# tuna2134/sbv2-api

Hardware: NVIDIA B200
Metric: audio-sec/sec (higher is better)
Workload: dtype f16 operands / f32 accumulate on tcgen05 (decoder, flow; text encoder with two-term fp16 splits); f32 elsewhere

## Files before the change

### sbv2-api_b200/csrc/umma_conv.h

```cpp
#pragma once
#include <cuda_fp16.h>

#include <map>
#include <vector>

#include "common.h"
#include "kernels.h"

struct sbv2_model;

namespace sbv2 {

constexpr int UMMA_GAP = 32;
constexpr int UMMA_TAIL_ROWS = 2304;
constexpr int UMMA_MAX_TAPS = 16;
constexpr int UMMA_MAX_GROUPS = 8;

struct HostConv {
  std::vector<float> w, b;
  int d0 = 0, d1 = 0, k = 1;
};

struct DecoderHostWeights {
  HostConv pre, cond, post;
  std::vector<HostConv> ups;
  std::vector<int> up_u;
  std::vector<std::vector<HostConv>> res_c1, res_c2;
  std::vector<std::vector<int>> res_dil;
  int per = 3;
  int gin = 512;
};

struct ConvLayer {
  __half* w = nullptr;
  float* bias = nullptr;
  int cin = 0, cout = 0, nb = 0, n_nblk = 1, taps = 1, kc = 64, nkc = 1, mt = 1, sps = 1, nstages = 2, nloads = 1, total_steps = 1;
  int a_slots = 1;
  int b_resident = 0;
  int n_groups = 1;
  int tap_shift[UMMA_MAX_GROUPS][UMMA_MAX_TAPS] = {{0}};
  int group_out_off[UMMA_MAX_GROUPS] = {0};
  int halo_lo = 0, halo_hi = 0;
  size_t smem = 0;
  int tmem_cols = 32;
  unsigned idesc = 0;
  float in_scale = 1.f, out_scale = 1.f;
};

ConvLayer make_conv1d_layer(sbv2_model* owner, const HostConv& c, int dil, int mt_pref, int nb_max = 256);
ConvLayer make_gated_conv1d_layer(sbv2_model* owner, const HostConv& c, int dil, int mt_pref, int* gate_half, std::vector<int>* perm);
ConvLayer make_upsample_layer(sbv2_model* owner, const HostConv& c, int u, int mt_pref);

struct Geom {
  int mul = 1;
  long long rows_tot = 0;
  std::vector<int> pstart, len;
  const int* d_pstart = nullptr;
  const int* d_len = nullptr;
  const int* d_prefix[5] = {nullptr, nullptr, nullptr, nullptr, nullptr};
  int n_tiles[5] = {0, 0, 0, 0, 0};
  std::map<int, std::pair<const int*, int>> extra;
  int max_len = 0;
};
struct BatchGeom {
  std::vector<Geom> g;
  const int* d_ystart = nullptr;
  const int* d_wstart = nullptr;
  const int* d_order = nullptr;
};
struct DBuf;
struct PinnedBuf;
BatchGeom build_geoms(sbv2_model* owner, DBuf& dev, PinnedBuf& pin, const std::vector<int>& ystart, const std::vector<int>& ylen,
                      const std::vector<int>& muls, const std::vector<std::vector<int>>* extra_heights = nullptr, bool pin_idle = false,
                      const std::vector<long long>* wstart = nullptr );

ConvLayer make_split_conv1d_layer(sbv2_model* owner, const HostConv& c, int dil, int mt_pref, int terms, int nb_max = 256);
void launch_split_planar(const LaunchCtx& ctx, __half* out, const float* in, int in_ld, int C, const int* d_start, const Geom& g,
                         int n_utt, int terms, float in_scale);
enum UAccum { UACC_NONE = 0, UACC_SET = 1, UACC_ADD = 2, UACC_FINAL = 3 };
struct ConvCall {
  const __half* in = nullptr;
  __half* out = nullptr;
  const __half* residual = nullptr;
  const __half* residual2 = nullptr;
  const __half* residual3 = nullptr;
  float out_div = 1.f;
  float* accum = nullptr;
  int accum_mode = UACC_NONE;
  float accum_div = 1.f;
  int act_out = ACT_NONE;
  bool act_on_accum = false;
  const float* bias_utt = nullptr;
  int bias_utt_ld = 0;
  int gate_half = 0;
  int out_mul = 1, out_off = 0;
  float* rm_out = nullptr;
  int rm_ld = 0;
  const int* rm_start = nullptr;
  __half* split_out = nullptr;
  float split_scale = 16.f;
  bool tmap = false;
  int cluster = 0;
  bool pair = false;
  bool splitk = false;
};
void launch_umma(const LaunchCtx& ctx, const ConvLayer& L, const Geom& gi, const Geom& go, const ConvCall& c, int n_utt);
void launch_zero_gaps(const LaunchCtx& ctx, __half* buf, int C, const Geom& g, int n_utt);
void launch_planar_cast(const LaunchCtx& ctx, __half* out, const float* in, int C, const Geom& g, int n_utt);
void launch_to_planar(const LaunchCtx& ctx, __half* out, const float* in, int in_ld, int C, const int* d_start, const Geom& g,
                      int n_utt, int act);
void launch_from_planar(const LaunchCtx& ctx, float* out, const __half* in, int C, const int* d_start, const Geom& g, int n_utt);

struct PairLayer {
  __half* w1 = nullptr;
  __half* w2 = nullptr;
  float* bias1 = nullptr;
  float* bias2 = nullptr;
  int c = 0, taps = 1, kc = 16, nkc = 1, mt = 1, t1rows = 128, t1pitch = 144, out_rows = 128, h1 = 0, h2 = 0;
  int shift1[UMMA_MAX_TAPS] = {0};
  int sps = 1, nstages = 1, nloads = 1, total_steps = 1, a_slots = 2, b_resident = 0;
  size_t smem = 0;
  int tmem_cols = 512;
  unsigned idesc = 0;
};
struct PairCall {
  const __half* in = nullptr;
  __half* out = nullptr;
  const __half* residual2 = nullptr;
  const __half* residual3 = nullptr;
  float out_div = 1.f;
  int act_out = ACT_LRELU;
};
bool make_pair_layer(sbv2_model* owner, const HostConv& c1, int dil, const HostConv& c2, PairLayer* out);
void launch_umma_pair(const LaunchCtx& ctx, const PairLayer& L, const Geom& g, const PairCall& c, int n_utt);

struct UmmaDecoder;
UmmaDecoder* umma_decoder_create(const DecoderHostWeights& w, sbv2_model* owner);
void umma_decoder_free(UmmaDecoder* d);
void umma_decoder_run(UmmaDecoder* d, sbv2_model* owner, const float* z, const float* g, int B,
                      const std::vector<int>& ystart, const std::vector<int>& ylen, float* wave,
                      const std::vector<long long>* wstart = nullptr);

}
```

### sbv2-api_b200/csrc/umma_pair.cu

```cuda
#include <cuda_fp16.h>

#include <algorithm>
#include <cstdlib>

#include "kernels.h"
#include "model.h"
#include "umma_conv.h"
#include "umma_device.cuh"

namespace sbv2 {
namespace {

constexpr int P_MAX_ASLOTS = 8, P_MAX_STAGES = 4, P_EPI_WARPS = 16, P_THREADS = 64 + 32 * P_EPI_WARPS + 32;
constexpr int P_B_PRODUCER_WARP = 2 + P_EPI_WARPS;
constexpr int P_SMEM_LIMIT = 227 * 1024;

struct PairArgs {
  __half* out;
  long long out_plane_stride;
  const __half* residual;
  const __half* residual2;
  const __half* residual3;
  float out_div;
  float* accum;
  int accum_mode, act_on_accum;
  float accum_div;
  int act_out;
  float act_slope;
  const __half* in;
  const __half* w1;
  const __half* w2;
  const float* bias1;
  const float* bias2;
  const int* tile_prefix;
  const int* pstart;
  const int* len;
  int n_utt, n_items;
  int c, taps, kc, nkc, mt, t1rows, t1pitch, out_rows, h1, h2;
  int shift1[UMMA_MAX_TAPS];
  int sps, nstages, nloads, total_steps, a_slots, b_resident;
  int has_res;
  int tmem_cols;
  unsigned idesc;
  long long* trace;
};

#define PTRACE(ev, itv)                                                                          \
  do {                                                                                            \
    if (p.trace != nullptr && blockIdx.x == 0 && (itv) < 64) p.trace[(itv) * 16 + (ev)] = clock64(); \
  } while (0)

struct PTile {
  int b, t0, len, pstart;
};
constexpr int P_TABLE_UTTS = 128;
struct PTables {
  const int* prefix;
  const int* len;
  const int* pstart;
};
__device__ __forceinline__ PTile locate_pair_item(const PairArgs& p, const PTables& tb, int item) {
  PTile ti;
  int lo = 0, hi = p.n_utt;
  while (hi - lo > 1) {
    const int mid = (lo + hi) >> 1;
    if (tb.prefix[mid] <= item) lo = mid;
    else hi = mid;
  }
  ti.b = lo;
  ti.t0 = (item - tb.prefix[lo]) * p.out_rows;
  ti.len = tb.len[lo];
  ti.pstart = tb.pstart[lo];
  return ti;
}

template <int C>
struct PairShape {
  static constexpr int c = C, mt = 128 / C, kc = C < 64 ? C : 64, nkc = C / kc, t1rows = 128 * mt, t1pitch = t1rows + 16;
};

template <int C>
__global__ void __launch_bounds__(P_THREADS, 1) umma_pair_kernel(const __grid_constant__ PairArgs p) {
  using K = PairShape<C>;
  extern __shared__ __align__(128) uint8_t smem[];
  const int warp = __shfl_sync(0xffffffffu, (int)(threadIdx.x >> 5), 0), lane = threadIdx.x & 31;
  const int RA = K::t1rows + 2 * p.h1;
  const int ppc = K::kc / 8;
  const uint32_t slot_bytes = (uint32_t)ppc * RA * 16;
  const uint32_t step_bytes = (uint32_t)K::c * K::kc * 2;
  const uint32_t stage_bytes = step_bytes * p.sps;
  const uint32_t t1_bytes = (uint32_t)(K::c / 8) * K::t1pitch * 16;
  const uint32_t sA = smem_u32(smem);
  const uint32_t sT1 = sA + ((slot_bytes * p.a_slots + 127u) & ~127u);
  const uint32_t sB = sT1 + 2 * t1_bytes;
  const uint32_t sBar = sB + (p.b_resident ? 2 * step_bytes * p.total_steps : stage_bytes * p.nstages);
  const uint32_t bar_af = sBar, bar_ae = bar_af + 8 * P_MAX_ASLOTS, bar_bf = bar_ae + 8 * P_MAX_ASLOTS, bar_be = bar_bf + 8 * P_MAX_STAGES,
                 bar_a1f = bar_be + 8 * P_MAX_STAGES, bar_a1e = bar_a1f + 16, bar_a2f = bar_a1e + 16, bar_a2e = bar_a2f + 16,
                 bar_t1r = bar_a2e + 16, bar_t1f = bar_t1r + 16;
  const uint32_t tmem_slot = bar_t1f + 16;
  volatile uint32_t* tmem_slot_ptr = reinterpret_cast<volatile uint32_t*>(smem + (tmem_slot - sA));
  float* bias_s = reinterpret_cast<float*>(smem + (sBar - sA) + 384);
  const int acc_cols = K::mt * K::c;

  if (threadIdx.x == 0) {
    for (int i = 0; i < p.a_slots; ++i) {
      mbar_init(bar_af + 8 * i, 1);
      mbar_init(bar_ae + 8 * i, 1);
    }
    for (int i = 0; i < P_MAX_STAGES; ++i) {
      mbar_init(bar_bf + 8 * i, 1);
      mbar_init(bar_be + 8 * i, 1);
    }
    for (int i = 0; i < 2; ++i) {
      mbar_init(bar_a1f + 8 * i, 1);
      mbar_init(bar_a1e + 8 * i, P_EPI_WARPS);
      mbar_init(bar_a2f + 8 * i, 1);
      mbar_init(bar_a2e + 8 * i, P_EPI_WARPS);
      mbar_init(bar_t1r + 8 * i, P_EPI_WARPS);
      mbar_init(bar_t1f + 8 * i, 1);
    }
    asm volatile("fence.mbarrier_init.release.cluster;" ::: "memory");
  }
  for (int i = threadIdx.x; i < 2 * K::c; i += P_THREADS) bias_s[i] = i < K::c ? p.bias1[i] : p.bias2[i - K::c];
  PTables tb{p.tile_prefix, p.len, p.pstart};
  if (p.n_utt <= P_TABLE_UTTS) {
    int* tab = reinterpret_cast<int*>(bias_s + 2 * K::c);
    for (int i = threadIdx.x; i <= p.n_utt; i += P_THREADS) tab[i] = p.tile_prefix[i];
    for (int i = threadIdx.x; i < p.n_utt; i += P_THREADS) {
      tab[p.n_utt + 1 + i] = p.len[i];
      tab[2 * p.n_utt + 1 + i] = p.pstart[i];
    }
    tb.prefix = tab;
    tb.len = tab + p.n_utt + 1;
    tb.pstart = tab + 2 * p.n_utt + 1;
  }
  if (warp == 1) {
    asm volatile("tcgen05.alloc.cta_group::1.sync.aligned.shared::cta.b32 [%0], %1;" ::"r"(tmem_slot), "r"((uint32_t)p.tmem_cols) : "memory");
    asm volatile("tcgen05.relinquish_alloc_permit.cta_group::1.sync.aligned;" ::: "memory");
  }
  tc_fence_before();
  __syncthreads();
  tc_fence_after();
  const uint32_t tmem_base = *tmem_slot_ptr;
  pdl_launch_dependents();
  pdl_wait();
  const int n_my = p.n_items > (int)blockIdx.x ? (p.n_items - 1 - (int)blockIdx.x) / (int)gridDim.x + 1 : 0;

  if (warp == 0) {
    if (lane == 0) {
      uint32_t a_it = 0;
      auto load_a_item = [&](int it) {
        const PTile ti = locate_pair_item(p, tb, (int)blockIdx.x + it * (int)gridDim.x);
        const long long in_row0 = (long long)ti.pstart + ti.t0 - p.h2 - p.h1;
        for (int kc = 0; kc < K::nkc; ++kc, ++a_it) {
          const uint32_t slot = a_it % p.a_slots;
          mbar_wait(bar_ae + 8 * slot, ((a_it / p.a_slots) & 1) ^ 1);
          mbar_expect_tx(bar_af + 8 * slot, slot_bytes);
          for (int q = 0; q < ppc; ++q) {
            const int plane = kc * ppc + q;
            bulk_g2s(sA + slot_bytes * slot + (uint32_t)q * RA * 16, p.in + (size_t)plane * p.out_plane_stride + in_row0 * 8, (uint32_t)RA * 16,
                     bar_af + 8 * slot);
          }
        }
      };
      for (int it = 0; it < n_my; ++it) load_a_item(it);
    }
  } else if (warp == P_B_PRODUCER_WARP) {
    if (lane == 0) {
      uint32_t b_it = 0;
      auto load_b_all = [&](const __half* w) {
        for (int i = 0; i < p.nloads; ++i, ++b_it) {
          const uint32_t st = b_it % p.nstages;
          mbar_wait(bar_be + 8 * st, ((b_it / p.nstages) & 1) ^ 1);
          const int first_step = i * p.sps;
          const int nsteps = min(p.sps, p.total_steps - first_step);
          const uint32_t bytes = step_bytes * nsteps;
          mbar_expect_tx(bar_bf + 8 * st, bytes);
          bulk_g2s(sB + stage_bytes * st, w + (size_t)first_step * (step_bytes / 2), bytes, bar_bf + 8 * st);
        }
      };
      if (p.b_resident && n_my > 0) {
        const uint32_t wb = step_bytes * p.total_steps;
        mbar_expect_tx(bar_bf, 2 * wb);
        bulk_g2s(sB, p.w1, wb, bar_bf);
        bulk_g2s(sB + wb, p.w2, wb, bar_bf);
      }
      if (!p.b_resident) {
        if (n_my > 0) load_b_all(p.w1);
        for (int it = 0; it < n_my; ++it) {
          if (it + 1 < n_my) load_b_all(p.w1);
          load_b_all(p.w2);
        }
      }
    }
  } else if (warp == 1) {
    const int k16 = K::kc / 16, mt = K::mt;
    const uint32_t c_u = (uint32_t)K::c, idesc = p.idesc;
    const uint64_t desc_hi = (uint64_t)(0x4000u | (128u >> 4)) << 32;
    const uint64_t a_desc0 = desc_hi | ((uint64_t)((uint32_t)RA & 0x3FFF) << 16);
    const uint64_t t_desc0 = desc_hi | ((uint64_t)((uint32_t)K::t1pitch & 0x3FFF) << 16);
    const uint64_t b_desc0 = desc_hi | ((uint64_t)((uint32_t)K::c & 0x3FFF) << 16);
    const uint32_t a_kstep = 2u * (uint32_t)RA, t_kstep = 2u * (uint32_t)K::t1pitch, b_kstep = 2u * (uint32_t)K::c;
    uint32_t a_slot_i = 0, a_par = 0, b_st = 0, b_par = 0;
    int b_si = 0;
    bool resident_ready = false;
    auto b_step_addr = [&](int conv, int step) -> uint32_t {
      if (p.b_resident) {
        if (!resident_ready) {
          mbar_wait(bar_bf, 0);
          resident_ready = true;
        }
        return sB + (uint32_t)conv * step_bytes * p.total_steps + step_bytes * step;
      }
      if (b_si == 0) mbar_wait(bar_bf + 8 * b_st, b_par);
      return sB + stage_bytes * b_st + step_bytes * b_si;
    };
    const bool leader = elect_one_sync() != 0;
    auto b_step_done = [&](int step) {
      if (p.b_resident) return;
      ++b_si;
      if (b_si == p.sps || step == p.total_steps - 1) {
        if (leader) tc_commit(bar_be + 8 * b_st);
        b_si = 0;
        if (++b_st == (uint32_t)p.nstages) {
          b_st = 0;
          b_par ^= 1;
        }
      }
    };
    auto issue_p1 = [&](int it, auto mtk) {
      constexpr int MT = decltype(mtk)::mt, K16 = decltype(mtk)::k16;
      const uint32_t buf = it & 1;
      mbar_wait(bar_a1e + 8 * buf, ((it >> 1) & 1) ^ 1);
      tc_fence_after();
      if (lane == 0) PTRACE(0, it);
      const uint32_t tacc0 = tmem_base + buf * acc_cols;
      int step = 0;
      for (int kc = 0; kc < K::nkc; ++kc) {
        mbar_wait(bar_af + 8 * a_slot_i, a_par);
        const uint64_t a_chunk = a_desc0 + ((sA + slot_bytes * a_slot_i) >> 4) + (uint32_t)p.h1;
        for (int tap = 0; tap < p.taps; ++tap, ++step) {
          const uint32_t b_addr = b_step_addr(0, step);
          const uint64_t a_tap = a_chunk + (int64_t)p.shift1[tap];
          const uint64_t b_d = b_desc0 + (b_addr >> 4);
          const uint32_t accf = step > 0 ? 1u : 0u;
          if (leader) issue_mmas<MT, K16>(tacc0, a_tap, b_d, a_kstep, b_kstep, c_u, idesc, accf);
          b_step_done(step);
        }
        if (leader) tc_commit(bar_ae + 8 * a_slot_i);
        if (++a_slot_i == (uint32_t)p.a_slots) {
          a_slot_i = 0;
          a_par ^= 1;
        }
      }
      if (leader) tc_commit(bar_a1f + 8 * buf);
      __syncwarp();
      if (lane == 0) PTRACE(1, it);
    };
    auto issue_p2 = [&](int it, auto mtk) {
      constexpr int MT = decltype(mtk)::mt, K16 = decltype(mtk)::k16;
      const uint32_t buf = it & 1;
      if (lane == 0) PTRACE(8, it);
      mbar_wait(bar_a2e + 8 * buf, ((it >> 1) & 1) ^ 1);
      if (lane == 0) PTRACE(9, it);
      mbar_wait(bar_t1r + 8 * buf, (it >> 1) & 1);
      tc_fence_after();
      if (lane == 0) PTRACE(2, it);
      const uint32_t tacc0 = tmem_base + (2 + buf) * acc_cols;
      const uint64_t t_tile = t_desc0 + ((sT1 + buf * t1_bytes) >> 4);
      int step = 0;
      for (int kc = 0; kc < K::nkc; ++kc) {
        const uint64_t t_chunk = t_tile + (uint32_t)(kc * ppc * K::t1pitch);
        for (int tap = 0; tap < p.taps; ++tap, ++step) {
          const uint32_t b_addr = b_step_addr(1, step);
          const uint64_t t_tap = t_chunk + (uint32_t)tap;
          const uint64_t b_d = b_desc0 + (b_addr >> 4);
          const uint32_t accf = step > 0 ? 1u : 0u;
          if (leader) issue_mmas<MT, K16>(tacc0, t_tap, b_d, t_kstep, b_kstep, c_u, idesc, accf);
          b_step_done(step);
        }
      }
      if (leader) {
        tc_commit(bar_a2f + 8 * buf);
        tc_commit(bar_t1f + 8 * buf);
      }
      __syncwarp();
      if (lane == 0) PTRACE(3, it);
    };
    auto run = [&](auto mtk) {
      if (n_my > 0) issue_p1(0, mtk);
      for (int it = 0; it < n_my; ++it) {
        if (it + 1 < n_my) issue_p1(it + 1, mtk);
        issue_p2(it, mtk);
      }
    };
    run(MtK<K::mt, K::kc / 16>{});
  } else {
    const int wq = warp & 3;
    const int part = (warp - 2) >> 2;
    constexpr int NPART = P_EPI_WARPS / 4;
    const float* b1s = bias_s;
    const float* b2s = bias_s + K::c;
    auto epi1 = [&](int it) {
      const uint32_t buf = it & 1;
      const PTile ti = locate_pair_item(p, tb, (int)blockIdx.x + it * (int)gridDim.x);
      mbar_wait(bar_a1f + 8 * buf, (it >> 1) & 1);
      mbar_wait(bar_t1f + 8 * buf, ((it >> 1) & 1) ^ 1);
      tc_fence_after();
      if (threadIdx.x == 64) PTRACE(4, it);
      if (threadIdx.x == 64 + 15 * 32) PTRACE(10, it);
      const uint32_t tacc0 = tmem_base + buf * acc_cols;
      uint8_t* t1 = smem + (sT1 - sA) + buf * t1_bytes;
      const int n_sub = K::mt * (K::c / 16);
      for (int sub = part; sub < n_sub; sub += NPART) {
        const int a = sub / (K::c / 16);
        const int c0 = (sub - a * (K::c / 16)) * 16;
        const int r = a * 128 + wq * 32 + lane;
        const int pos = ti.t0 - p.h2 + r;
        const bool inside = pos >= 0 && pos < ti.len;
        uint32_t v[16];
        tc_ld16(tacc0 + ((uint32_t)(wq * 32) << 16) + (uint32_t)(a * K::c + c0), v);
        tc_wait_ld();
#pragma unroll
        for (int pl = 0; pl < 2; ++pl) {
          const float4 bb0 = *reinterpret_cast<const float4*>(b1s + c0 + 8 * pl), bb1 = *reinterpret_cast<const float4*>(b1s + c0 + 8 * pl + 4);
          float f[8];
          f[0] = __uint_as_float(v[8 * pl + 0]) + bb0.x; f[1] = __uint_as_float(v[8 * pl + 1]) + bb0.y;
          f[2] = __uint_as_float(v[8 * pl + 2]) + bb0.z; f[3] = __uint_as_float(v[8 * pl + 3]) + bb0.w;
          f[4] = __uint_as_float(v[8 * pl + 4]) + bb1.x; f[5] = __uint_as_float(v[8 * pl + 5]) + bb1.y;
          f[6] = __uint_as_float(v[8 * pl + 6]) + bb1.z; f[7] = __uint_as_float(v[8 * pl + 7]) + bb1.w;
          uint4 o = make_uint4(0, 0, 0, 0);
          if (inside) {
            __half2* oh = reinterpret_cast<__half2*>(&o);
#pragma unroll
            for (int e = 0; e < 4; ++e) oh[e] = __floats2half2_rn(fmaxf(f[2 * e], f[2 * e] * 0.1f), fmaxf(f[2 * e + 1], f[2 * e + 1] * 0.1f));
          }
          *reinterpret_cast<uint4*>(t1 + ((size_t)((c0 >> 3) + pl) * K::t1pitch + r) * 16) = o;
        }
      }
      asm volatile("fence.proxy.async.shared::cta;" ::: "memory");
      tc_fence_before();
      __syncwarp();
      if (threadIdx.x == 64) PTRACE(5, it);
      if (threadIdx.x == 64 + 15 * 32) PTRACE(11, it);
      if (lane == 0) {
        asm volatile("mbarrier.arrive.shared::cta.b64 _, [%0];" ::"r"(bar_a1e + 8 * buf) : "memory");
        asm volatile("mbarrier.arrive.shared::cta.b64 _, [%0];" ::"r"(bar_t1r + 8 * buf) : "memory");
      }
    };
    auto epi2 = [&](int it) {
      const uint32_t buf = it & 1;
      const PTile ti = locate_pair_item(p, tb, (int)blockIdx.x + it * (int)gridDim.x);
      mbar_wait(bar_a2f + 8 * buf, (it >> 1) & 1);
      tc_fence_after();
      if (threadIdx.x == 64) PTRACE(6, it);
      if (threadIdx.x == 64 + 15 * 32) PTRACE(12, it);
      const uint32_t tacc0 = tmem_base + (2 + buf) * acc_cols;
      const bool wide = (K::c % 32 == 0) && p.has_res != 3;
      const int nch = wide ? 32 : 16;
      const int per_acc = K::c / nch;
      const int n_sub = K::mt * per_acc;
      for (int sub = part; sub < n_sub; sub += NPART) {
        const int a = sub / per_acc;
        const int c0 = (sub - a * per_acc) * nch;
        const int m = a * 128 + wq * 32 + lane;
        const int t = ti.t0 + m;
        const bool valid = m < p.out_rows && t < ti.len;
        const long long orow = (long long)ti.pstart + t;
        const uint32_t taddr = tacc0 + ((uint32_t)(wq * 32) << 16) + (uint32_t)(a * K::c + c0);
        if (p.has_res == 3) epilogue_item<16, false, 3>(p, taddr, valid, orow, c0, b2s + c0);
        else if (wide) epilogue_item<32, false, 1>(p, taddr, valid, orow, c0, b2s + c0);
        else epilogue_item<16, false, 1>(p, taddr, valid, orow, c0, b2s + c0);
      }
      tc_fence_before();
      __syncwarp();
      if (threadIdx.x == 64) PTRACE(7, it);
      if (threadIdx.x == 64 + 15 * 32) PTRACE(13, it);
      if (lane == 0) asm volatile("mbarrier.arrive.shared::cta.b64 _, [%0];" ::"r"(bar_a2e + 8 * buf) : "memory");
    };
    if (n_my > 0) epi1(0);
    for (int it = 0; it < n_my; ++it) {
      if (it + 1 < n_my) epi1(it + 1);
      epi2(it);
    }
  }
  tc_fence_before();
  __syncthreads();
  if (warp == 1) {
    asm volatile("tcgen05.dealloc.cta_group::1.sync.aligned.b32 %0, %1;" ::"r"(tmem_base), "r"((uint32_t)p.tmem_cols) : "memory");
  }
}

uint16_t f2h_(float f) { return __half_as_ushort(__float2half_rn(f)); }

__half* pack_conv(sbv2_model* owner, const HostConv& c, int kc) {
  const int C = c.d0, k = c.k, nkc = C / kc;
  std::vector<uint16_t> pk(size_t(C) * C * k);
  size_t o = 0;
  for (int q = 0; q < nkc; ++q)
    for (int tap = 0; tap < k; ++tap)
      for (int pl = 0; pl < kc / 8; ++pl)
        for (int n = 0; n < C; ++n)
          for (int e = 0; e < 8; ++e) pk[o++] = f2h_(c.w[(size_t(n) * C + q * kc + pl * 8 + e) * k + tap]);
  return static_cast<__half*>(owner->upload_bytes(pk.data(), pk.size() * 2));
}

}

long long* g_pair_trace = nullptr;

bool make_pair_layer(sbv2_model* owner, const HostConv& c1, int dil, const HostConv& c2, PairLayer* out) {
  PairLayer L;
  const int C = c1.d0, k = c1.k;
  if (c1.d1 != C || c2.d0 != C || c2.d1 != C || c2.k != k || k % 2 == 0 || k > UMMA_MAX_TAPS) return false;
  if (C != 16 && C != 32 && C != 64 && C != 128) return false;
  L.c = C;
  L.taps = k;
  L.h1 = dil * (k - 1) / 2;
  L.h2 = (k - 1) / 2;
  if (L.h1 + L.h2 > UMMA_GAP) return false;
  for (int j = 0; j < k; ++j) L.shift1[j] = (j - (k - 1) / 2) * dil;
  L.kc = C % 64 == 0 ? 64 : (C % 32 == 0 ? 32 : 16);
  L.nkc = C / L.kc;
  L.total_steps = k * L.nkc;
  L.mt = 128 / C;
  if (L.mt < 1) return false;
  L.t1rows = 128 * L.mt;
  L.t1pitch = L.t1rows + 16;
  L.out_rows = L.t1rows - 2 * L.h2;
  const size_t step_bytes = size_t(C) * L.kc * 2;
  const size_t w_bytes = step_bytes * L.total_steps;
  const size_t slot = size_t(L.kc / 8) * (L.t1rows + 2 * L.h1) * 16;
  const size_t t1 = size_t(C / 8) * L.t1pitch * 16;
  const size_t misc = 384 + size_t(2) * C * 4 + 256 + size_t(3 * P_TABLE_UTTS + 1) * 4;
  const size_t budget = P_SMEM_LIMIT;
  const int min_slots = std::max(2, std::min(2 * L.nkc, P_MAX_ASLOTS));
  if (2 * w_bytes + slot * min_slots + 2 * t1 + misc <= budget) {
    L.b_resident = 1;
    L.sps = L.total_steps;
    L.nloads = 1;
    L.nstages = 1;
    L.a_slots = min_slots;
    while (L.a_slots < P_MAX_ASLOTS && L.a_slots < 3 * L.nkc && 2 * w_bytes + slot * (L.a_slots + 1) + 2 * t1 + misc <= budget) ++L.a_slots;
    L.smem = ((slot * L.a_slots + 127) & ~size_t(127)) + 2 * t1 + 2 * w_bytes + misc;
  } else {
    L.b_resident = 0;
    L.sps = int(std::max<size_t>(1, (16 * 1024) / step_bytes));
    L.sps = std::min(L.sps, L.total_steps);
    L.nloads = (L.total_steps + L.sps - 1) / L.sps;
    const size_t stage_bytes = step_bytes * L.sps;
    bool placed = false;
    for (int ns = P_MAX_STAGES; ns >= 2 && !placed; --ns)
      for (int slots = P_MAX_ASLOTS; slots >= min_slots && !placed; --slots) {
        const size_t sm = ((slot * slots + 127) & ~size_t(127)) + 2 * t1 + stage_bytes * ns + misc;
        if (sm <= budget) {
          L.nstages = ns;
          L.a_slots = slots;
          L.smem = sm;
          placed = true;
        }
      }
    if (!placed) return false;
  }
  L.tmem_cols = 512;
  L.idesc = (1u << 4) | ((unsigned)(C >> 3) << 17) | ((unsigned)(128 >> 4) << 24);
  L.w1 = pack_conv(owner, c1, L.kc);
  L.w2 = pack_conv(owner, c2, L.kc);
  L.bias1 = owner->upload_f32(c1.b);
  L.bias2 = owner->upload_f32(c2.b);
  *out = L;
  return true;
}

void launch_umma_pair(const LaunchCtx& ctx, const PairLayer& L, const Geom& g, const PairCall& c, int n_utt) {
  static PerDeviceOnce attr_once;
  attr_once.run([&] {
    CUDA_CHECK(cudaFuncSetAttribute(umma_pair_kernel<16>, cudaFuncAttributeMaxDynamicSharedMemorySize, P_SMEM_LIMIT));
    CUDA_CHECK(cudaFuncSetAttribute(umma_pair_kernel<32>, cudaFuncAttributeMaxDynamicSharedMemorySize, P_SMEM_LIMIT));
    CUDA_CHECK(cudaFuncSetAttribute(umma_pair_kernel<64>, cudaFuncAttributeMaxDynamicSharedMemorySize, P_SMEM_LIMIT));
    CUDA_CHECK(cudaFuncSetAttribute(umma_pair_kernel<128>, cudaFuncAttributeMaxDynamicSharedMemorySize, P_SMEM_LIMIT));
  });
  auto it = g.extra.find(L.out_rows);
  if (it == g.extra.end()) fail(SBV2_ERR_INTERNAL, "geometry lacks the tile table for a fused ResBlock pair");
  PairArgs a;
  a.out = c.out;
  a.out_plane_stride = g.rows_tot * 8;
  a.residual = c.in;
  a.residual2 = c.residual2;
  a.residual3 = c.residual3;
  a.out_div = c.out_div;
  a.accum = nullptr;
  a.accum_mode = UACC_NONE;
  a.act_on_accum = 0;
  a.accum_div = 1.f;
  a.act_out = c.act_out;
  a.act_slope = c.act_out == ACT_LRELU ? 0.1f : (c.act_out == ACT_LRELU01 ? 0.01f : (c.act_out == ACT_RELU ? 0.f : 1.f));
  a.in = c.in;
  a.w1 = L.w1;
  a.w2 = L.w2;
  a.bias1 = L.bias1;
  a.bias2 = L.bias2;
  a.tile_prefix = it->second.first;
  a.pstart = g.d_pstart;
  a.len = g.d_len;
  a.n_utt = n_utt;
  a.n_items = it->second.second;
  a.c = L.c;
  a.taps = L.taps;
  a.kc = L.kc;
  a.nkc = L.nkc;
  a.mt = L.mt;
  a.t1rows = L.t1rows;
  a.t1pitch = L.t1pitch;
  a.out_rows = L.out_rows;
  a.h1 = L.h1;
  a.h2 = L.h2;
  for (int i = 0; i < UMMA_MAX_TAPS; ++i) a.shift1[i] = L.shift1[i];
  a.sps = L.sps;
  a.nstages = L.nstages;
  a.nloads = L.nloads;
  a.total_steps = L.total_steps;
  a.a_slots = L.a_slots;
  a.b_resident = L.b_resident;
  a.has_res = c.residual2 ? 3 : 1;
  a.tmem_cols = L.tmem_cols;
  a.idesc = L.idesc;
  a.trace = g_pair_trace;
  if (a.n_items <= 0) return;
  static int num_sms = 0;
  if (num_sms == 0) {
    int dev = 0;
    CUDA_CHECK(cudaGetDevice(&dev));
    CUDA_CHECK(cudaDeviceGetAttribute(&num_sms, cudaDevAttrMultiProcessorCount, dev));
  }
  int grid = std::min(a.n_items, num_sms);
  if (g_pair_trace != nullptr) {
    if (const char* e = getenv("SBV2_B200_PAIR_GRID")) grid = std::max(1, std::min(grid, atoi(e)));
  }
  void (*kernel)(PairArgs) = nullptr;
  switch (L.c) {
    case 16: kernel = umma_pair_kernel<16>; break;
    case 32: kernel = umma_pair_kernel<32>; break;
    case 64: kernel = umma_pair_kernel<64>; break;
    case 128: kernel = umma_pair_kernel<128>; break;
    default: fail(SBV2_ERR_INTERNAL, "fused ResBlock pair: unsupported channel count");
  }
  launch_pdl(ctx.pdl, kernel, dim3(grid), dim3(P_THREADS), L.smem, ctx.stream, a);
  ctx.count();
}

}
```

Measured before the change: 9036.

## Fold time rows into N dimension for second conv of small-channel ResBlock pairs

For channel counts 16 and 32, the second convolution of the fused ResBlock pair now folds R consecutive time rows into the MMA N dimension. The intermediate T1 tile is stored row-interleaved by phase, and the weights are repacked into a block-Toeplitz layout with R+k-1 steps. This replaces k narrow-N MMAs per K chunk with fewer, wider MMAs (N = R*C) over fewer M tiles, to raise tensor-core utilisation on these tiny-channel layers. It costs extra shared memory for the larger folded weights, padding of the T1 tile, and zero-initialisation of that padding. Configurations that do not fit in resident mode are rejected.

```diff
diff --git a/sbv2-api_b200/csrc/umma_conv.h b/sbv2-api_b200/csrc/umma_conv.h
--- a/sbv2-api_b200/csrc/umma_conv.h
+++ b/sbv2-api_b200/csrc/umma_conv.h
@@ -116,8 +116,7 @@
   __half* w2 = nullptr;
   float* bias1 = nullptr;
   float* bias2 = nullptr;
-  int c = 0, taps = 1, kc = 16, nkc = 1, mt = 1, t1rows = 128, t1pitch = 144, out_rows = 128, h1 = 0, h2 = 0;
-  int shift1[UMMA_MAX_TAPS] = {0};
+  int c = 0, taps = 1, kc = 16, nkc = 1, mt = 1, t1rows = 128, t1pitch = 144, out_rows = 128, h1 = 0, h2 = 0;  int shift1[UMMA_MAX_TAPS] = {0};
   int sps = 1, nstages = 1, nloads = 1, total_steps = 1, a_slots = 2, b_resident = 0;
   size_t smem = 0;
   int tmem_cols = 512;
diff --git a/sbv2-api_b200/csrc/umma_pair.cu b/sbv2-api_b200/csrc/umma_pair.cu
--- a/sbv2-api_b200/csrc/umma_pair.cu
+++ b/sbv2-api_b200/csrc/umma_pair.cu
@@ -74,9 +74,14 @@
   return ti;
 }
 
+__host__ __device__ constexpr int pair_fold(int C) { return C == 16 ? 4 : (C == 32 ? 2 : 1); }
+__host__ __device__ constexpr int pair_t1pad(int R) { return R == 4 ? 10 : (R == 2 ? 12 : 16); }
+__host__ __device__ constexpr unsigned pair_idesc(int n) { return (1u << 4) | ((unsigned)(n >> 3) << 17) | ((unsigned)(128 >> 4) << 24); }
+
 template <int C>
 struct PairShape {
-  static constexpr int c = C, mt = 128 / C, kc = C < 64 ? C : 64, nkc = C / kc, t1rows = 128 * mt, t1pitch = t1rows + 16;
+  static constexpr int c = C, mt = 128 / C, kc = C < 64 ? C : 64, nkc = C / kc, t1rows = 128 * mt;
+  static constexpr int r = pair_fold(C), n2 = r * C, mt2 = mt / r, t1pitch = t1rows / r + pair_t1pad(r);
 };
 
 template <int C>
@@ -89,11 +94,14 @@
   const uint32_t slot_bytes = (uint32_t)ppc * RA * 16;
   const uint32_t step_bytes = (uint32_t)K::c * K::kc * 2;
   const uint32_t stage_bytes = step_bytes * p.sps;
-  const uint32_t t1_bytes = (uint32_t)(K::c / 8) * K::t1pitch * 16;
+  const uint32_t w1_bytes = step_bytes * p.total_steps;
+  const uint32_t step2_bytes = (uint32_t)K::n2 * K::kc * 2;
+  const uint32_t w2_bytes = step2_bytes * (K::r == 1 ? p.total_steps : K::r + p.taps - 1);
+  const uint32_t t1_bytes = (uint32_t)(K::c / 8) * K::r * K::t1pitch * 16;
   const uint32_t sA = smem_u32(smem);
   const uint32_t sT1 = sA + ((slot_bytes * p.a_slots + 127u) & ~127u);
   const uint32_t sB = sT1 + 2 * t1_bytes;
-  const uint32_t sBar = sB + (p.b_resident ? 2 * step_bytes * p.total_steps : stage_bytes * p.nstages);
+  const uint32_t sBar = sB + (p.b_resident ? w1_bytes + w2_bytes : stage_bytes * p.nstages);
   const uint32_t bar_af = sBar, bar_ae = bar_af + 8 * P_MAX_ASLOTS, bar_bf = bar_ae + 8 * P_MAX_ASLOTS, bar_be = bar_bf + 8 * P_MAX_STAGES,
                  bar_a1f = bar_be + 8 * P_MAX_STAGES, bar_a1e = bar_a1f + 16, bar_a2f = bar_a1e + 16, bar_a2e = bar_a2f + 16,
                  bar_t1r = bar_a2e + 16, bar_t1f = bar_t1r + 16;
@@ -133,6 +141,12 @@
     tb.prefix = tab;
     tb.len = tab + p.n_utt + 1;
     tb.pstart = tab + 2 * p.n_utt + 1;
+  }
+  if constexpr (K::r > 1) {
+    constexpr int rows = K::t1rows / K::r, pad = K::t1pitch - rows, n_planes = 2 * (K::c / 8) * K::r;
+    uint4* t1z = reinterpret_cast<uint4*>(smem + (sT1 - sA));
+    for (int i = threadIdx.x; i < n_planes * pad; i += P_THREADS) t1z[(i / pad) * K::t1pitch + rows + i % pad] = make_uint4(0, 0, 0, 0);
+    asm volatile("fence.proxy.async.shared::cta;" ::: "memory");
   }
   if (warp == 1) {
     asm volatile("tcgen05.alloc.cta_group::1.sync.aligned.shared::cta.b32 [%0], %1;" ::"r"(tmem_slot), "r"((uint32_t)p.tmem_cols) : "memory");
@@ -180,10 +194,9 @@
         }
       };
       if (p.b_resident && n_my > 0) {
-        const uint32_t wb = step_bytes * p.total_steps;
-        mbar_expect_tx(bar_bf, 2 * wb);
-        bulk_g2s(sB, p.w1, wb, bar_bf);
-        bulk_g2s(sB + wb, p.w2, wb, bar_bf);
+        mbar_expect_tx(bar_bf, w1_bytes + w2_bytes);
+        bulk_g2s(sB, p.w1, w1_bytes, bar_bf);
+        bulk_g2s(sB + w1_bytes, p.w2, w2_bytes, bar_bf);
       }
       if (!p.b_resident) {
         if (n_my > 0) load_b_all(p.w1);
@@ -198,9 +211,11 @@
     const uint32_t c_u = (uint32_t)K::c, idesc = p.idesc;
     const uint64_t desc_hi = (uint64_t)(0x4000u | (128u >> 4)) << 32;
     const uint64_t a_desc0 = desc_hi | ((uint64_t)((uint32_t)RA & 0x3FFF) << 16);
-    const uint64_t t_desc0 = desc_hi | ((uint64_t)((uint32_t)K::t1pitch & 0x3FFF) << 16);
+    const uint64_t t_desc0 = desc_hi | ((uint64_t)((uint32_t)(K::r * K::t1pitch) & 0x3FFF) << 16);
     const uint64_t b_desc0 = desc_hi | ((uint64_t)((uint32_t)K::c & 0x3FFF) << 16);
-    const uint32_t a_kstep = 2u * (uint32_t)RA, t_kstep = 2u * (uint32_t)K::t1pitch, b_kstep = 2u * (uint32_t)K::c;
+    const uint64_t b2_desc0 = desc_hi | ((uint64_t)((uint32_t)K::n2 & 0x3FFF) << 16);
+    const uint32_t a_kstep = 2u * (uint32_t)RA, t_kstep = 2u * (uint32_t)(K::r * K::t1pitch), b_kstep = 2u * (uint32_t)K::c,
+                   b2_kstep = 2u * (uint32_t)K::n2;
     uint32_t a_slot_i = 0, a_par = 0, b_st = 0, b_par = 0;
     int b_si = 0;
     bool resident_ready = false;
@@ -210,7 +225,8 @@
           mbar_wait(bar_bf, 0);
           resident_ready = true;
         }
-        return sB + (uint32_t)conv * step_bytes * p.total_steps + step_bytes * step;
+        if constexpr (K::r == 1) return sB + (uint32_t)conv * step_bytes * p.total_steps + step_bytes * step;
+        return conv == 0 ? sB + step_bytes * step : sB + w1_bytes + step2_bytes * step;
       }
       if (b_si == 0) mbar_wait(bar_bf + 8 * b_st, b_par);
       return sB + stage_bytes * b_st + step_bytes * b_si;
@@ -268,16 +284,25 @@
       if (lane == 0) PTRACE(2, it);
       const uint32_t tacc0 = tmem_base + (2 + buf) * acc_cols;
       const uint64_t t_tile = t_desc0 + ((sT1 + buf * t1_bytes) >> 4);
-      int step = 0;
-      for (int kc = 0; kc < K::nkc; ++kc) {
-        const uint64_t t_chunk = t_tile + (uint32_t)(kc * ppc * K::t1pitch);
-        for (int tap = 0; tap < p.taps; ++tap, ++step) {
-          const uint32_t b_addr = b_step_addr(1, step);
-          const uint64_t t_tap = t_chunk + (uint32_t)tap;
-          const uint64_t b_d = b_desc0 + (b_addr >> 4);
-          const uint32_t accf = step > 0 ? 1u : 0u;
-          if (leader) issue_mmas<MT, K16>(tacc0, t_tap, b_d, t_kstep, b_kstep, c_u, idesc, accf);
-          b_step_done(step);
+      if constexpr (K::r == 1) {
+        int step = 0;
+        for (int kc = 0; kc < K::nkc; ++kc) {
+          const uint64_t t_chunk = t_tile + (uint32_t)(kc * ppc * K::t1pitch);
+          for (int tap = 0; tap < p.taps; ++tap, ++step) {
+            const uint32_t b_addr = b_step_addr(1, step);
+            const uint64_t t_tap = t_chunk + (uint32_t)tap;
+            const uint64_t b_d = b_desc0 + (b_addr >> 4);
+            const uint32_t accf = step > 0 ? 1u : 0u;
+            if (leader) issue_mmas<MT, K16>(tacc0, t_tap, b_d, t_kstep, b_kstep, c_u, idesc, accf);
+            b_step_done(step);
+          }
+        }
+      } else {
+        constexpr uint32_t idesc2 = pair_idesc(K::n2);
+        for (int s = 0; s < K::r + p.taps - 1; ++s) {
+          const uint64_t t_s = t_tile + (uint32_t)((s % K::r) * K::t1pitch + s / K::r);
+          const uint64_t b_d = b2_desc0 + (b_step_addr(1, s) >> 4);
+          if (leader) issue_mmas<K::mt2, K16>(tacc0, t_s, b_d, t_kstep, b2_kstep, (uint32_t)K::n2, idesc2, s > 0 ? 1u : 0u);
         }
       }
       if (leader) {
@@ -335,7 +360,7 @@
 #pragma unroll
             for (int e = 0; e < 4; ++e) oh[e] = __floats2half2_rn(fmaxf(f[2 * e], f[2 * e] * 0.1f), fmaxf(f[2 * e + 1], f[2 * e + 1] * 0.1f));
           }
-          *reinterpret_cast<uint4*>(t1 + ((size_t)((c0 >> 3) + pl) * K::t1pitch + r) * 16) = o;
+          *reinterpret_cast<uint4*>(t1 + ((size_t)(((c0 >> 3) + pl) * K::r + r % K::r) * K::t1pitch + r / K::r) * 16) = o;
         }
       }
       asm volatile("fence.proxy.async.shared::cta;" ::: "memory");
@@ -361,13 +386,13 @@
       const int per_acc = K::c / nch;
       const int n_sub = K::mt * per_acc;
       for (int sub = part; sub < n_sub; sub += NPART) {
-        const int a = sub / per_acc;
-        const int c0 = (sub - a * per_acc) * nch;
-        const int m = a * 128 + wq * 32 + lane;
+        const int ar = sub / per_acc;
+        const int c0 = (sub - ar * per_acc) * nch;
+        const int m = ((ar / K::r) * 128 + wq * 32 + lane) * K::r + ar % K::r;
         const int t = ti.t0 + m;
         const bool valid = m < p.out_rows && t < ti.len;
         const long long orow = (long long)ti.pstart + t;
-        const uint32_t taddr = tacc0 + ((uint32_t)(wq * 32) << 16) + (uint32_t)(a * K::c + c0);
+        const uint32_t taddr = tacc0 + ((uint32_t)(wq * 32) << 16) + (uint32_t)(ar * K::c + c0);
         if (p.has_res == 3) epilogue_item<16, false, 3>(p, taddr, valid, orow, c0, b2s + c0);
         else if (wide) epilogue_item<32, false, 1>(p, taddr, valid, orow, c0, b2s + c0);
         else epilogue_item<16, false, 1>(p, taddr, valid, orow, c0, b2s + c0);
@@ -402,6 +427,20 @@
       for (int pl = 0; pl < kc / 8; ++pl)
         for (int n = 0; n < C; ++n)
           for (int e = 0; e < 8; ++e) pk[o++] = f2h_(c.w[(size_t(n) * C + q * kc + pl * 8 + e) * k + tap]);
+  return static_cast<__half*>(owner->upload_bytes(pk.data(), pk.size() * 2));
+}
+
+__half* pack_conv_folded(sbv2_model* owner, const HostConv& c, int R) {
+  const int C = c.d0, k = c.k, N = R * C;
+  std::vector<uint16_t> pk(size_t(R + k - 1) * C * N, 0);
+  size_t o = 0;
+  for (int s = 0; s < R + k - 1; ++s)
+    for (int pl = 0; pl < C / 8; ++pl)
+      for (int n = 0; n < N; ++n)
+        for (int e = 0; e < 8; ++e, ++o) {
+          const int tap = s - n / C;
+          if (tap >= 0 && tap < k) pk[o] = f2h_(c.w[(size_t(n % C) * C + pl * 8 + e) * k + tap]);
+        }
   return static_cast<__half*>(owner->upload_bytes(pk.data(), pk.size() * 2));
 }
 
@@ -426,23 +465,29 @@
   L.mt = 128 / C;
   if (L.mt < 1) return false;
   L.t1rows = 128 * L.mt;
-  L.t1pitch = L.t1rows + 16;
+  const int R = pair_fold(C);
+  if ((R + k - 2) / R > pair_t1pad(R)) return false;
+  L.t1pitch = L.t1rows / R + pair_t1pad(R);
   L.out_rows = L.t1rows - 2 * L.h2;
   const size_t step_bytes = size_t(C) * L.kc * 2;
   const size_t w_bytes = step_bytes * L.total_steps;
+  const size_t w2_bytes = R == 1 ? w_bytes : size_t(R) * C * C * 2 * (R + k - 1);
   const size_t slot = size_t(L.kc / 8) * (L.t1rows + 2 * L.h1) * 16;
-  const size_t t1 = size_t(C / 8) * L.t1pitch * 16;
+  const size_t t1 = size_t(C / 8) * R * L.t1pitch * 16;
   const size_t misc = 384 + size_t(2) * C * 4 + 256 + size_t(3 * P_TABLE_UTTS + 1) * 4;
   const size_t budget = P_SMEM_LIMIT;
   const int min_slots = std::max(2, std::min(2 * L.nkc, P_MAX_ASLOTS));
-  if (2 * w_bytes + slot * min_slots + 2 * t1 + misc <= budget) {
+  if (w_bytes + w2_bytes + slot * min_slots + 2 * t1 + misc <= budget) {
     L.b_resident = 1;
     L.sps = L.total_steps;
     L.nloads = 1;
     L.nstages = 1;
     L.a_slots = min_slots;
-    while (L.a_slots < P_MAX_ASLOTS && L.a_slots < 3 * L.nkc && 2 * w_bytes + slot * (L.a_slots + 1) + 2 * t1 + misc <= budget) ++L.a_slots;
-    L.smem = ((slot * L.a_slots + 127) & ~size_t(127)) + 2 * t1 + 2 * w_bytes + misc;
+    while (L.a_slots < P_MAX_ASLOTS && L.a_slots < 3 * L.nkc && w_bytes + w2_bytes + slot * (L.a_slots + 1) + 2 * t1 + misc <= budget)
+      ++L.a_slots;
+    L.smem = ((slot * L.a_slots + 127) & ~size_t(127)) + 2 * t1 + w_bytes + w2_bytes + misc;
+  } else if (R > 1) {
+    return false;
   } else {
     L.b_resident = 0;
     L.sps = int(std::max<size_t>(1, (16 * 1024) / step_bytes));
@@ -463,9 +508,9 @@
     if (!placed) return false;
   }
   L.tmem_cols = 512;
-  L.idesc = (1u << 4) | ((unsigned)(C >> 3) << 17) | ((unsigned)(128 >> 4) << 24);
+  L.idesc = pair_idesc(C);
   L.w1 = pack_conv(owner, c1, L.kc);
-  L.w2 = pack_conv(owner, c2, L.kc);
+  L.w2 = R == 1 ? pack_conv(owner, c2, L.kc) : pack_conv_folded(owner, c2, R);
   L.bias1 = owner->upload_f32(c1.b);
   L.bias2 = owner->upload_f32(c2.b);
   *out = L;
```

Result: no change. 9014 (median of 6 runs) (-0.2%).
